# chenxy99/Scanpaths

Measured on AMD Instinct MI355X. Metric: images/sec/GPU (AiR train step, bs=32, 320x512) at 1/2/4/8 MI355X, higher is better.
Workload: dtype f32; 1 GPU; AiR supervised train step (fwd+loss+bwd+clip+Adam), resnet50, T=16, 320x512, per-GPU batch 32; global_batch=32, parallelism=dp1

## Files before the change

### scanpaths_amd/csrc/conv_f16x2.hip

```cpp
#include "common.h"
#include <algorithm>
#include <cstdlib>

typedef _Float16 f16x8 __attribute__((ext_vector_type(8)));

namespace {

#define SP_GLDS16(src, dst)                                                                                      \
    __builtin_amdgcn_global_load_lds((const __attribute__((address_space(1))) void*)(src),                       \
                                     (__attribute__((address_space(3))) void*)(dst), 16, 0, 0)

constexpr int HBM = 256, HBN = 128, HBK = 32;
constexpr int HA_BYTES = HBM * 128;
constexpr int HB_BYTES = HBN * 128;
constexpr int HSTAGE = HA_BYTES + HB_BYTES;
constexpr int HNSTAGE = 3;
constexpr int HCHUNK_KT = 8;
constexpr int HALO_W = 64, HALO_ROWSLOTS = HALO_W + 2, HALO_NSLOT = 6 * HALO_ROWSLOTS;
constexpr int HALO_PIECES = (HALO_NSLOT + 7) / 8;
constexpr int HALO_A_BYTES = HALO_PIECES * 1024;
constexpr int HALO_LDS = 2 * HALO_A_BYTES + 3 * HB_BYTES;

struct H2Args {
    const uint16_t* X;
    const uint16_t* W;
    const float* bias;
    float* C;
    const float* sx;
    const float* sw;
    int sw_rows;
    int64_t M;
    int Hi, Wi, Kc;
    int ldx;
    int Ho, Wo, Nout, ldc;
    int KH, KW, stride, pad, dil;
    int64_t ldwb;
    int64_t w_bstride;
    int rows_per_batch;
    int ncblk, nkt, tiles_n;
    float alpha;
    int beta, relu;
    uint32_t x_bytes, w_bytes;
    const float* l_xg;
    const float* l_cprev;
    const float* l_spcol;
    const float* l_wc;
    float* l_gates;
    float* l_c;
    float* l_h;
    unsigned* l_hamax;
    uint16_t* l_hplanes;
    float* l_hscale;
    float l_hbound;
    int lC, lP, lKP;
    int l_probe;
    double* st_partial;
    float* st_mm;
    const int* row_last;
    int row_step;
    int row_nimg;
};

__device__ __forceinline__ float h2_sigmoid(float x) { return sp_sigmoid(x); }
__device__ __forceinline__ int halo_swz(int slot) { return ((slot >> 1) & 3) << 1; }

template <int MODE, int NPROD, bool CBM, bool LSTM = false, bool HALO = false, int DBG = 0>
__global__ __launch_bounds__(512, 2) void h2_kernel(H2Args p) {
    static_assert(!LSTM || MODE == 0, "the LSTM epilogue belongs to the forward build");
    static_assert(!HALO || (CBM && NPROD == 3 && DBG == 0), "the halo build extends the channel-block-major schedule only");
    extern __shared__ __attribute__((aligned(16))) unsigned char smem[];
    constexpr bool LSTM_T = LSTM;
    const int t = threadIdx.x;
    const int lane = t & 63;
    const int wave = __builtin_amdgcn_readfirstlane(t >> 6);
    const int wm = wave >> 1, wn = wave & 1;

#ifdef SP_TIMING_VARIANTS
    const int probe = p.l_probe;
    if ((probe >> 8) && blockIdx.x < 256) {
        const int G = (probe >> 8) & 15, step_us = 2 * ((probe >> 12) & 31);
        const long long wait = (long long)((blockIdx.x >> 3) % G) * step_us * 100;
        const long long t0 = __builtin_amdgcn_s_memrealtime();
        while ((long long)__builtin_amdgcn_s_memrealtime() - t0 < wait) __builtin_amdgcn_s_sleep(32);
    }
#else
    constexpr int probe = 0;
#endif
    const float sx_dev = p.sx[0], sw_dev = p.sw_rows ? 1.f : p.sw[0];
    int tn, tmi;
    bool mapped = false;
    if constexpr (MODE == 1 && !LSTM) {
        if (p.row_nimg > 0) {
            const int mine = lane < p.row_nimg ? p.row_last[lane] : -1;
            const uint64_t lm = __ballot(lane < p.row_nimg && mine >= p.row_step);
            const uint64_t all = p.row_nimg == 64 ? ~0ull : ((1ull << p.row_nimg) - 1ull);
            const int tps = (p.Ho * p.Wo) / HBM;
            const int nlive = __popcll(lm);
            const int nl = nlive * tps * p.tiles_n;
            const int bid = blockIdx.x;
            uint64_t mask;
            int tml;
            if (bid < nl) {
                supertile_map(xcd_remap(bid, nl), nlive * tps, p.tiles_n, tml, tn, CBM);
                mask = lm;
            } else {
                tn = (bid - nl) % p.tiles_n;
                tml = (bid - nl) / p.tiles_n;
                mask = all & ~lm;
            }
            for (int k = tml / tps; k > 0; --k) mask &= mask - 1ull;
            tmi = (__ffsll((unsigned long long)mask) - 1) * tps + tml % tps;
            mapped = true;
        }
    }
    if (!mapped) supertile_map(xcd_remap(blockIdx.x, gridDim.x), gridDim.x / p.tiles_n, p.tiles_n, tmi, tn, CBM);
    const int64_t m0 = (int64_t)tmi * HBM;
    const int n0 = LSTM ? tn * 32 : tn * HBN;
    if constexpr (!LSTM) {
        if (p.row_last != nullptr) {
            const int howo = MODE == 1 ? p.Ho * p.Wo : p.rows_per_batch;
            const int img = (int)(m0 / howo);
            if (howo % HBM == 0 && m0 < p.M && p.row_last[img] < p.row_step) {
// ... 36 lines not shown
            a_px[j] = xo * p.stride - p.pad;
        } else {
            a_py[j] = yo + p.pad;
            a_px[j] = xo + p.pad;
        }
    }
    uint32_t b_voff[2];
    bool b_ok[2];
#pragma unroll
    for (int j = 0; j < 2; ++j) {
        const int idx = t + 512 * j;
        const int row = idx >> 3, pos = idx & 7;
        const int c8 = (pos ^ ((row >> 1) & 7)) * 16;
        if constexpr (LSTM) {
            const int ch = n0 + (row >> 6) * 16 + (row & 15);
            b_ok[j] = ch < p.lC;
            b_voff[j] = b_ok[j] ? (uint32_t)((int64_t)(((row >> 4) & 3) * p.lC + ch) * p.ldwb + c8) : 0u;
        } else {
            b_ok[j] = (n0 + row) < p.Nout;
            b_voff[j] = b_ok[j] ? (uint32_t)((int64_t)(n0 + row) * p.ldwb + c8) : 0u;
        }
    }
    const unsigned char* Wl = reinterpret_cast<const unsigned char*>(p.W);
    uint32_t w_left = p.w_bytes;
    if constexpr (!CBM) {
        if (p.w_bstride) {
            const int64_t off = (m0 / p.rows_per_batch) * p.w_bstride;
            Wl += off;
            w_left -= (uint32_t)off;
        }
    }
    int ld_ky = 0, ld_kx = 0, ld_cblk = 0, ld_kt = 0;
    uint32_t a_voff[4];
    bool a_ok[4];
    const int rowbytes = p.ldx * 4;
    uint32_t a_base0[4], a_mask[4];
    if constexpr (CBM && !HALO) {
#pragma unroll
        for (int j = 0; j < 4; ++j) {
            a_base0[j] = (uint32_t)(a_boff[j] + a_py[j] * p.Wi + a_px[j]) * (uint32_t)rowbytes + (uint32_t)a_c8[j];
            uint32_t msk = 0;
            for (int ky = 0; ky < p.KH; ++ky)
                for (int kx = 0; kx < p.KW; ++kx) {
                    const int iy = MODE == 0 ? a_py[j] + ky * p.dil : a_py[j] - ky * p.dil;
                    const int ix = MODE == 0 ? a_px[j] + kx * p.dil : a_px[j] - kx * p.dil;
                    if (a_rowok[j] && (unsigned)iy < (unsigned)p.Hi && (unsigned)ix < (unsigned)p.Wi) msk |= 1u << (ky * p.KW + kx);
                }
            a_mask[j] = msk;
        }
    }
    int ld_tap = 0;
    uint32_t h_off[7];
    uint32_t h_valid = 0;
    const int h_npieces = HALO ? (HALO_PIECES - wave + 7) / 8 : 0;
    if constexpr (HALO) {
        const int img = (int)((uint32_t)m0 / (uint32_t)HoWo);
        const int y0 = (int)(((uint32_t)m0 - (uint32_t)img * (uint32_t)HoWo) / (uint32_t)p.Wo);
#pragma unroll
        for (int j = 0; j < 7; ++j) {
            const int slot = (wave + 8 * j) * 8 + (lane >> 3), pos = lane & 7;
            const int br = slot / HALO_ROWSLOTS, sx = slot - br * HALO_ROWSLOTS;
            const int y = y0 - 1 + br, x = sx - 1;
            const bool ok = slot < HALO_NSLOT && (unsigned)y < (unsigned)p.Hi && (unsigned)x < (unsigned)p.Wi && m0 < p.M;
            h_off[j] = ok ? (uint32_t)((img * p.Hi + y) * p.Wi + x) * (uint32_t)rowbytes + (uint32_t)((pos ^ halo_swz(slot)) * 16) : 0u;
            h_valid |= ok ? (1u << j) : 0u;
        }
    }
    int h_cb = 0;
    auto issue_block = [&]() {
        if constexpr (HALO) {
            unsigned char* stA = smem + (h_cb & 1) * HALO_A_BYTES;
            const uint32_t koffA = (uint32_t)h_cb * 128u;
            const unsigned char* baseA = reinterpret_cast<const unsigned char*>(p.X) + koffA;
            const uint32_t zrelA = p.x_bytes - koffA;
#pragma unroll
            for (int j = 0; j < 7; ++j)
                if (j < h_npieces) SP_GLDS16(baseA + (((h_valid >> j) & 1u) ? h_off[j] : zrelA), stA + (wave + 8 * j) * 1024);
            ++h_cb;
        }
    };

    auto tap_update = [&]() {
#pragma unroll
        for (int j = 0; j < 4; ++j) {
            bool ok = a_rowok[j];
            int iy, ix;
            if (MODE == 0) {
                iy = a_py[j] + ld_ky * p.dil;
                ix = a_px[j] + ld_kx * p.dil;
                ok = ok && (unsigned)iy < (unsigned)p.Hi && (unsigned)ix < (unsigned)p.Wi;
            } else {
                const int ty = a_py[j] - ld_ky * p.dil, tx = a_px[j] - ld_kx * p.dil;
                ok = ok && ty >= 0 && tx >= 0;
                if (p.stride == 1) {
                    iy = ty;
                    ix = tx;
                } else {
                    iy = ty / p.stride;
                    ix = tx / p.stride;
                    ok = ok && (iy * p.stride == ty) && (ix * p.stride == tx);
                }
                ok = ok && iy < p.Hi && ix < p.Wi;
            }
            a_ok[j] = ok;
            a_voff[j] = ok ? (uint32_t)(a_boff[j] + iy * p.Wi + ix) * (uint32_t)rowbytes + (uint32_t)a_c8[j] : 0u;
        }
    };

    auto issue_tile = [&](int stage) {
        unsigned char* st = smem + stage * HSTAGE;
        if constexpr (HALO) {
            unsigned char* stB = smem + 2 * HALO_A_BYTES + stage * HB_BYTES;
            const uint32_t koffB = (uint32_t)(ld_tap * p.ncblk + ld_cblk) * 128u;
            const unsigned char* baseB = reinterpret_cast<const unsigned char*>(p.W) + koffB;
            const uint32_t zrelB = p.w_bytes - koffB;
#pragma unroll
            for (int j = 0; j < 2; ++j) SP_GLDS16(baseB + (b_ok[j] ? b_voff[j] : zrelB), stB + (wave + 8 * j) * 1024);
            if (++ld_tap == 9) {
                ld_tap = 0;
                ++ld_cblk;
            }
            return;
        }
        if constexpr (CBM) {
            const int step = (ld_ky * p.Wi + ld_kx) * p.dil;
            const uint32_t delta = (uint32_t)(MODE == 0 ? step : -step) * (uint32_t)rowbytes;
            const uint32_t koffA = (uint32_t)ld_cblk * 128u;
            const unsigned char* baseA = reinterpret_cast<const unsigned char*>(p.X) + koffA;
            const uint32_t zrelA = p.x_bytes - koffA;
#pragma unroll
            for (int j = 0; j < 4; ++j)
                SP_GLDS16(baseA + (((a_mask[j] >> ld_tap) & 1u) ? a_base0[j] + delta : zrelA), st + (wave + 8 * j) * 1024);
            const uint32_t koffB = (uint32_t)(ld_tap * p.ncblk + ld_cblk) * 128u;
            const unsigned char* baseB = reinterpret_cast<const unsigned char*>(p.W) + koffB;
            const uint32_t zrelB = p.w_bytes - koffB;
#pragma unroll
            for (int j = 0; j < 2; ++j) SP_GLDS16(baseB + (b_ok[j] ? b_voff[j] : zrelB), st + HA_BYTES + (wave + 8 * j) * 1024);
            ++ld_tap;
            if (++ld_kx == p.KW) {
                ld_kx = 0;
                if (++ld_ky == p.KH) {
                    ld_ky = 0;
                    ld_tap = 0;
                    ++ld_cblk;
                }
            }
            return;
        }
        if (ld_cblk == 0) tap_update();
        const uint32_t koffA = (uint32_t)ld_cblk * 128u;
        const unsigned char* baseA = reinterpret_cast<const unsigned char*>(p.X) + koffA;
        const uint32_t zrelA = p.x_bytes - koffA;
#pragma unroll
        for (int j = 0; j < 4; ++j) SP_GLDS16(baseA + (a_ok[j] ? a_voff[j] : zrelA), st + (wave + 8 * j) * 1024);
        const uint32_t koffB = (uint32_t)ld_kt * 128u;
        const unsigned char* baseB = Wl + koffB;
        const uint32_t zrelB = w_left - koffB;
#pragma unroll
        for (int j = 0; j < 2; ++j) SP_GLDS16(baseB + (b_ok[j] ? b_voff[j] : zrelB), st + HA_BYTES + (wave + 8 * j) * 1024);
        ++ld_kt;
        if (++ld_cblk == p.ncblk) {
            ld_cblk = 0;
            if (++ld_kx == p.KW) {
                ld_kx = 0;
                ++ld_ky;
            }
        }
    };

    const int l16 = lane & 15, g4 = lane >> 4;
    float pre_sw[4] = {1.f, 1.f, 1.f, 1.f};
    if constexpr (!LSTM && !HALO) {
        if (p.sw_rows) {
            int64_t r0 = 0;
            if constexpr (!CBM) {
                if (p.w_bstride) r0 = (m0 / p.rows_per_batch) * (int64_t)p.Nout;
            }
#pragma unroll
            for (int j = 0; j < 4; ++j) {
                const int n = n0 + wn * 64 + j * 16 + l16;
                if (n < p.Nout) pre_sw[j] = p.sw[r0 + n];
            }
        }
    }
    const int rot = (l16 >> 1) & 7;
    int offA[2], offB[2];
#pragma unroll
    for (int pl = 0; pl < 2; ++pl) {
        const int pos = ((g4 >> 1) * 4 + pl * 2 + (g4 & 1)) ^ rot;
        offA[pl] = (wm * 64 + l16) * 128 + pos * 16;
        offB[pl] = HA_BYTES + (wn * 64 + l16) * 128 + pos * 16;
    }

    const int h_slot0 = wm * HALO_ROWSLOTS + l16;
    const int h_chunk = (g4 >> 1) * 4 + (g4 & 1);
    int rd_tap = 0, rd_cb = 0;
    f32x4 tot4[4][4], acc4[4][4];
#pragma unroll
    for (int i = 0; i < 4; ++i)
#pragma unroll
        for (int j = 0; j < 4; ++j)
#pragma unroll
            for (int r = 0; r < 4; ++r) {
                tot4[i][j][r] = 0.f;
                acc4[i][j][r] = 0.f;
            }

    constexpr bool do_load = DBG != 1 && DBG != 3, do_mma = DBG != 2 && DBG != 9, do_lds = DBG != 3 && DBG != 9;
    constexpr bool do_bar = DBG != 3;
    int issued = 0;
    if constexpr (HALO) issue_block();
    if (do_load)
        for (; issued < HNSTAGE - 1 && issued < p.nkt; ++issued) issue_tile(issued);
    if (issued >= 2) {
        if constexpr (HALO) asm volatile("s_waitcnt vmcnt(2)" ::: "memory");
        else asm volatile("s_waitcnt vmcnt(6)" ::: "memory");
    } else {
        asm volatile("s_waitcnt vmcnt(0)" ::: "memory");
    }
    __builtin_amdgcn_s_barrier();

    f16x8 af[2][2][2], bf[2][2][2];
    auto read_frags = [&](int stage_, int kt_) {
        const unsigned char* st = smem + stage_ * HSTAGE;
        if constexpr (!do_lds) {
#pragma unroll
            for (int kk = 0; kk < 2; ++kk)
#pragma unroll
                for (int i = 0; i < 2; ++i)
#pragma unroll
                    for (int pl = 0; pl < 2; ++pl) {
                        f16x8 z;
#pragma unroll
                        for (int e = 0; e < 8; ++e) z[e] = (_Float16)(float)(kt_ + e + lane);
                        af[kk][i][pl] = z;
                        bf[kk][i][pl] = z;
                    }
        } else if constexpr (HALO) {
            const int ky = rd_tap / 3, kx = rd_tap - 3 * ky;
            const int slot = h_slot0 + (MODE == 0 ? ky * HALO_ROWSLOTS + kx : (2 - ky) * HALO_ROWSLOTS + 2 - kx);
            const int sw = halo_swz(slot);
            const unsigned char* stA = smem + (rd_cb & 1) * HALO_A_BYTES + slot * 128;
            const unsigned char* stB = smem + 2 * HALO_A_BYTES + stage_ * HB_BYTES - HA_BYTES;
            const int oa0 = ((h_chunk) ^ sw) * 16, oa1 = ((h_chunk + 2) ^ sw) * 16;
#pragma unroll
            for (int kk = 0; kk < 2; ++kk)
#pragma unroll
                for (int i = 0; i < 2; ++i) {
                    af[kk][i][0] = *reinterpret_cast<const f16x8*>(stA + oa0 + (2 * kk + i) * 16 * 128);
                    af[kk][i][1] = *reinterpret_cast<const f16x8*>(stA + oa1 + (2 * kk + i) * 16 * 128);
                    bf[kk][i][0] = *reinterpret_cast<const f16x8*>(stB + offB[0] + (2 * kk + i) * 16 * 128);
                    bf[kk][i][1] = *reinterpret_cast<const f16x8*>(stB + offB[1] + (2 * kk + i) * 16 * 128);
                }
            if (++rd_tap == 9) {
                rd_tap = 0;
                ++rd_cb;
            }
        } else {
#pragma unroll
            for (int kk = 0; kk < 2; ++kk)
#pragma unroll
                for (int i = 0; i < 2; ++i)
#pragma unroll
                    for (int pl = 0; pl < (NPROD == 3 ? 2 : 1); ++pl) {
                        af[kk][i][pl] = *reinterpret_cast<const f16x8*>(st + offA[pl] + (2 * kk + i) * 16 * 128);
                        bf[kk][i][pl] = *reinterpret_cast<const f16x8*>(st + offB[pl] + (2 * kk + i) * 16 * 128);
                    }
        }
    };
    auto mma_group = [&](int kk) {
        if constexpr (do_mma) {
#pragma unroll
            for (int i = 0; i < 2; ++i)
#pragma unroll
                for (int j = 0; j < 4; ++j) {
                    f32x4& a4 = acc4[2 * kk + i][j];
                    if constexpr (LSTM_T) {
                        if constexpr (NPROD == 3) {
                            a4 = __builtin_amdgcn_mfma_f32_16x16x32_f16(bf[j >> 1][j & 1][1], af[kk][i][0], a4, 0, 0, 0);
                            a4 = __builtin_amdgcn_mfma_f32_16x16x32_f16(bf[j >> 1][j & 1][0], af[kk][i][1], a4, 0, 0, 0);
                        }
                        a4 = __builtin_amdgcn_mfma_f32_16x16x32_f16(bf[j >> 1][j & 1][0], af[kk][i][0], a4, 0, 0, 0);
                        continue;
                    }
                    if constexpr (NPROD == 3) {
                        a4 = __builtin_amdgcn_mfma_f32_16x16x32_f16(af[kk][i][0], bf[j >> 1][j & 1][1], a4, 0, 0, 0);
                        a4 = __builtin_amdgcn_mfma_f32_16x16x32_f16(af[kk][i][1], bf[j >> 1][j & 1][0], a4, 0, 0, 0);
                    }
                    a4 = __builtin_amdgcn_mfma_f32_16x16x32_f16(af[kk][i][0], bf[j >> 1][j & 1][0], a4, 0, 0, 0);
                }
        } else {
#pragma unroll
            for (int i = 0; i < 2; ++i)
#pragma unroll
                for (int pl = 0; pl < 2; ++pl) {
                    const f16x8 x0 = af[kk][i][pl], x1 = bf[kk][i][pl];
                    asm volatile("" ::"v"(x0), "v"(x1));
                }
        }
    };
    auto fold = [&](int kt_) {
        if (((kt_ + 1) & (HCHUNK_KT - 1)) == 0) {
#pragma unroll
            for (int i = 0; i < 4; ++i)
#pragma unroll
                for (int j = 0; j < 4; ++j) {
                    tot4[i][j] += acc4[i][j];
#pragma unroll
                    for (int r = 0; r < 4; ++r) acc4[i][j][r] = 0.f;
                }
        }
    };
    auto wait_barrier = [&](int kt_) {
        if (kt_ + 2 < p.nkt) asm volatile("s_waitcnt vmcnt(6)" ::: "memory");
        else asm volatile("s_waitcnt vmcnt(0)" ::: "memory");
        asm volatile("s_waitcnt lgkmcnt(0)" ::: "memory");
        if constexpr (do_bar) __builtin_amdgcn_s_barrier();
    };
    auto prev_stage = [](int st_) { return st_ == 0 ? HNSTAGE - 1 : st_ - 1; };

    int stage = 0;
    const bool late = wave >= 4;
    if (late) __builtin_amdgcn_s_setprio(1);
    if constexpr (HALO) {
        int cur_tap = 0, cur_cb = 0;
        auto halo_issue = [&](int kt_) {
            if (kt_ + HNSTAGE - 1 < p.nkt) issue_tile(prev_stage(stage));
            if (cur_tap == 0 && cur_cb + 1 < p.ncblk) issue_block();
        };
        auto halo_wait = [&](int kt_) {
            if (kt_ + 2 < p.nkt) {
                if (cur_tap <= 1 && cur_cb + 1 < p.ncblk) {
                    if (h_npieces == 7) asm volatile("s_waitcnt vmcnt(9)" ::: "memory");
                    else asm volatile("s_waitcnt vmcnt(8)" ::: "memory");
                } else {
                    asm volatile("s_waitcnt vmcnt(2)" ::: "memory");
                }
            } else {
                asm volatile("s_waitcnt vmcnt(0)" ::: "memory");
            }
            asm volatile("s_waitcnt lgkmcnt(0)" ::: "memory");
            __builtin_amdgcn_s_barrier();
            if (++cur_tap == 9) {
                cur_tap = 0;
                ++cur_cb;
            }
        };
        if (!late) {
            for (int kt = 0; kt < p.nkt; ++kt) {
                read_frags(stage, kt);
                halo_issue(kt);
                mma_group(0);
                mma_group(1);
                fold(kt);
                halo_wait(kt);
                stage = (stage == HNSTAGE - 1) ? 0 : stage + 1;
            }
        } else {
            for (int kt = 0; kt < p.nkt; ++kt) {
                if (kt > 0) {
                    mma_group(0);
                    mma_group(1);
                    fold(kt - 1);
                }
                read_frags(stage, kt);
                halo_issue(kt);
                halo_wait(kt);
                stage = (stage == HNSTAGE - 1) ? 0 : stage + 1;
            }
            mma_group(0);
            mma_group(1);
            fold(p.nkt - 1);
        }
    } else if (!late) {
        for (int kt = 0; kt < p.nkt; ++kt) {
            const bool pre = do_load && kt + HNSTAGE - 1 < p.nkt;
            if (!CBM && pre) issue_tile(prev_stage(stage));
            read_frags(stage, kt);
            if (CBM && pre) issue_tile(prev_stage(stage));
            mma_group(0);
            mma_group(1);
            fold(kt);
            wait_barrier(kt);
            stage = (stage == HNSTAGE - 1) ? 0 : stage + 1;
        }
    } else {
        for (int kt = 0; kt < p.nkt; ++kt) {
            const bool pre = do_load && kt + HNSTAGE - 1 < p.nkt;
            if (kt > 0) {
                mma_group(0);
                mma_group(1);
                fold(kt - 1);
            }
            read_frags(stage, kt);
            if (pre) issue_tile(prev_stage(stage));
            wait_barrier(kt);
            stage = (stage == HNSTAGE - 1) ? 0 : stage + 1;
        }
        mma_group(0);
        mma_group(1);
        fold(p.nkt - 1);
    }
    if (late) __builtin_amdgcn_s_setprio(0);

    const float isx = 1.f / sx_dev, isw = 1.f / sw_dev;
    int64_t swrow0 = 0;
    if constexpr (!CBM) {
        if (p.w_bstride) swrow0 = (m0 / p.rows_per_batch) * (int64_t)p.Nout;
    }
    if constexpr (LSTM_T) {
        if (probe & 4) return;
        const bool nt_st = probe & 8, nt_ld = probe & 16;
        auto st4 = [&](float* dst, const float4& v) {
            const f32x4 x = {v.x, v.y, v.z, v.w};
            if (nt_st) __builtin_nontemporal_store(x, reinterpret_cast<f32x4*>(dst));
            else *reinterpret_cast<f32x4*>(dst) = x;
        };
        auto ld4 = [&](const float* src) {
            const f32x4 x = nt_ld ? __builtin_nontemporal_load(reinterpret_cast<const f32x4*>(src)) : *reinterpret_cast<const f32x4*>(src);
            return make_float4(x[0], x[1], x[2], x[3]);
        };
        const int KP = p.lKP, C = p.lC;
        const int b = (int)(m0 / p.lP);
        const int chb = n0 + wn * 16 + 4 * g4;
// ... 230 lines not shown
                    if (p.beta) {
                        const float4 o = *dst;
                        v.x += o.x; v.y += o.y; v.z += o.z; v.w += o.w;
                    }
                    if (p.relu) {
                        v.x = fmaxf(v.x, 0.f); v.y = fmaxf(v.y, 0.f); v.z = fmaxf(v.z, 0.f); v.w = fmaxf(v.w, 0.f);
                    }
                    *dst = v;
                }
            }
        }
        if (stats) {
            asm volatile("s_waitcnt lgkmcnt(0)" ::: "memory");
            __builtin_amdgcn_s_barrier();
            double* sh_s = reinterpret_cast<double*>(smem);
            float* sh_m = reinterpret_cast<float*>(smem + 4 * HBN * 2 * sizeof(double));
#pragma unroll
            for (int j = 0; j < 4; ++j) {
#pragma unroll
                for (int off = 16; off <= 32; off <<= 1) {
                    cs[j] += __shfl_xor(cs[j], off);
                    cq[j] += __shfl_xor(cq[j], off);
                    cmn[j] = fminf(cmn[j], __shfl_xor(cmn[j], off));
                    cmx[j] = fmaxf(cmx[j], __shfl_xor(cmx[j], off));
                }
                if (g4 == 0) {
                    const int col = wn * 64 + j * 16 + l16;
                    sh_s[(wm * HBN + col) * 2 + 0] = cs[j];
                    sh_s[(wm * HBN + col) * 2 + 1] = cq[j];
                    sh_m[(wm * HBN + col) * 2 + 0] = cmn[j];
                    sh_m[(wm * HBN + col) * 2 + 1] = cmx[j];
                }
            }
            asm volatile("s_waitcnt lgkmcnt(0)" ::: "memory");
            __builtin_amdgcn_s_barrier();
            if (t < HBN && n0 + t < p.Nout) {
                double a = 0.0, b = 0.0;
                float mn = INFINITY, mx = -INFINITY;
#pragma unroll
                for (int w = 0; w < 4; ++w) {
                    a += sh_s[(w * HBN + t) * 2 + 0];
                    b += sh_s[(w * HBN + t) * 2 + 1];
                    mn = fminf(mn, sh_m[(w * HBN + t) * 2 + 0]);
                    mx = fmaxf(mx, sh_m[(w * HBN + t) * 2 + 1]);
                }
                const int64_t g = m0 / HBM;
                p.st_partial[(g * 2 + 0) * p.Nout + n0 + t] = a;
                p.st_partial[(g * 2 + 1) * p.Nout + n0 + t] = b;
                p.st_mm[(g * 2 + 0) * p.Nout + n0 + t] = mn;
                p.st_mm[(g * 2 + 1) * p.Nout + n0 + t] = mx;
            }
        }
    }
}

struct HWArgs {
    const uint16_t* X;
    const uint16_t* dY;
    float* out;
    const float* sx;
    const float* sy;
    int sx_vec, sy_vec;
    int64_t M;
    int Hi, Wi, Ci, Ho, Wo, Co;
    int ldy;
    int Nvalid;
    int batched;
    int KH, KW, stride, pad, dil;
    int Ntot, ldo, tiles_n, splits;
    int64_t rows_per_split, slab_stride;
    float alpha;
    int beta;
    uint32_t x_bytes, y_bytes;
    const int* row_last;
    int row_step;
};

constexpr int HWA_ROW = 1024, HWB_ROW = 512;
constexpr int HWA_BYTES = 32 * HWA_ROW;
constexpr int HWB_BYTES = 32 * HWB_ROW;
constexpr int HWSTAGE = HWA_BYTES + HWB_BYTES;

typedef short short4v __attribute__((ext_vector_type(4)));

__device__ __forceinline__ f16x8 tr_pair_h(const unsigned char* base, int off0, int off1) {
    const short4v lo = __builtin_amdgcn_ds_read_tr16_b64_v4i16((__attribute__((address_space(3))) short4v*)(base + off0));
    const short4v hi = __builtin_amdgcn_ds_read_tr16_b64_v4i16((__attribute__((address_space(3))) short4v*)(base + off1));
    typedef short short8v __attribute__((ext_vector_type(8)));
    short8v v = __builtin_shufflevector(lo, hi, 0, 1, 2, 3, 4, 5, 6, 7);
    return __builtin_bit_cast(f16x8, v);
}

__device__ __forceinline__ int rot4(int q) { return 2 * (q & 1) + 8 * (q >> 1); }
__device__ __forceinline__ int swz16(int r) { return rot4(r & 3) + 4 * ((r >> 3) & 1); }
__device__ __forceinline__ int permA16(int j) { return ((j & 0x0c) << 2) | ((j & 0x30) >> 2) | (j & 3); }
__device__ __forceinline__ int permB16(int j) { return ((j & 0x0c) << 1) | ((j & 0x10) >> 2) | (j & 3); }
__device__ __forceinline__ int unpermB16(int x) { return ((x & 0x18) >> 1) | ((x & 0x04) << 2) | (x & 3); }

template <int NPROD, int DBG = 0>
__global__ __launch_bounds__(512, 2) void hw_kernel(HWArgs p) {
    constexpr bool do_load = DBG != 1 && DBG != 3 && DBG != 6, do_mma = DBG != 2 && DBG != 5 && DBG != 6, do_lds = DBG != 3 && DBG != 5 && DBG != 9;
    constexpr bool load_a = DBG != 8, load_b = DBG != 7;
    constexpr bool do_bar = DBG != 3;
    extern __shared__ __attribute__((aligned(16))) unsigned char smem[];
    const int t = threadIdx.x;
    const int lane = t & 63;
// ... 777 lines not shown
        const int c4 = c0 + cgi;
        float4 m = make_float4(0.f, 0.f, 0.f, 0.f);
        if (rr < rpb && c4 < C4)
            for (int64_t r = (int64_t)blockIdx.x * rpb + rr; r < rows; r += (int64_t)gridDim.x * rpb) {
                const float4 v = reinterpret_cast<const float4*>(x + r * C)[c4];
                m.x = fmaxf(m.x, fabsf(v.x)); m.y = fmaxf(m.y, fabsf(v.y)); m.z = fmaxf(m.z, fabsf(v.z)); m.w = fmaxf(m.w, fabsf(v.w));
            }
        __syncthreads();
        sh[threadIdx.x] = m;
        __syncthreads();
        if (rr == 0 && c4 < C4) {
            for (int k = 1; k < rpb; ++k) {
                const float4 o = sh[k * cg_per + cgi];
                m.x = fmaxf(m.x, o.x); m.y = fmaxf(m.y, o.y); m.z = fmaxf(m.z, o.z); m.w = fmaxf(m.w, o.w);
            }
            reinterpret_cast<float4*>(partial + (int64_t)blockIdx.x * C)[c4] = m;
        }
    }
}
__global__ __launch_bounds__(256) void colamax_final_kernel(const float* partial, int nblk, int C, float* col_scale) {
    __shared__ float sh[256];
    const int c = blockIdx.x * 32 + (threadIdx.x & 31), rg = threadIdx.x >> 5;
    float m = 0.f;
    if (c < C)
        for (int b = rg; b < nblk; b += 8) m = fmaxf(m, partial[(int64_t)b * C + c]);
    sh[threadIdx.x] = m;
    __syncthreads();
    if (rg == 0 && c < C) {
#pragma unroll
        for (int k = 1; k < 8; ++k) m = fmaxf(m, sh[k * 32 + (threadIdx.x & 31)]);
        col_scale[c] = m > 0.f ? scale_of(__float_as_uint(m)) : 0x1p100f;
    }
}

__global__ __launch_bounds__(256) void split2_cols_kernel(const float* x, int64_t n4, int C, const float* col_scale, uint16_t* out) {
    const int lane = threadIdx.x & 63;
    const int C4 = C / 4;
    const int64_t stride = (int64_t)gridDim.x * blockDim.x;
    for (int64_t base = (int64_t)blockIdx.x * blockDim.x + (threadIdx.x & ~63); base < n4; base += stride) {
        const int64_t i = base + lane;
        const bool live = i < n4;
        const float4 v = live ? reinterpret_cast<const float4*>(x)[i] : make_float4(0.f, 0.f, 0.f, 0.f);
        const float4 sc = live ? reinterpret_cast<const float4*>(col_scale)[i % C4] : make_float4(1.f, 1.f, 1.f, 1.f);
        ushort4 a, b;
        split2(v.x, sc.x, a.x, b.x);
        split2(v.y, sc.y, a.y, b.y);
        split2(v.z, sc.z, a.z, b.z);
        split2(v.w, sc.w, a.w, b.w);
        store_planes_quad(out, i, live, a, b);
    }
    if (blockIdx.x == 0 && threadIdx.x < 8) reinterpret_cast<uint2*>(out + 8 * n4)[threadIdx.x] = make_uint2(0u, 0u);
}

template <int MODE, int NPROD, bool CBM, bool LSTM = false, bool HALO = false, int DBG = 0>
int launch_h2(const H2Args& a, hipStream_t s) {
    auto kern = h2_kernel<MODE, NPROD, CBM, LSTM, HALO, DBG>;
    constexpr int lds = HALO ? HALO_LDS : HNSTAGE * HSTAGE;
    static bool attr_set = false;
    if (!attr_set) {
        (void)hipFuncSetAttribute(reinterpret_cast<const void*>(kern), hipFuncAttributeMaxDynamicSharedMemorySize, lds);
        attr_set = true;
    }
    const int64_t grid = sp_cdiv(a.M, HBM) * a.tiles_n;
    if (grid <= 0 || grid > 0x7fffffff) return SP_EINVAL;
    hipLaunchKernelGGL(kern, dim3((unsigned)grid), dim3(512), lds, s, a);
    SP_LAUNCH_CHECK();
    return SP_OK;
}

template <int NPROD, int DBG = 0>
int launch_hw(const HWArgs& a, int Co, hipStream_t s) {
    auto kern = hw_kernel<NPROD, DBG>;
    static bool attr_set = false;
    if (!attr_set) {
        (void)hipFuncSetAttribute(reinterpret_cast<const void*>(kern), hipFuncAttributeMaxDynamicSharedMemorySize, HNSTAGE * HWSTAGE);
        attr_set = true;
    }
    const int64_t grid = sp_cdiv(Co, 256) * a.tiles_n;
    hipLaunchKernelGGL(kern, dim3((unsigned)grid, (unsigned)a.splits), dim3(512), HNSTAGE * HWSTAGE, s, a);
    SP_LAUNCH_CHECK();
    return SP_OK;
}

int launch_amax(const float* x, int64_t n, unsigned* amax, hipStream_t s) {
    SP_RESET_AMAX(amax, s);
    const int64_t n4 = n / 4;
    const int blocks = (int)std::max<int64_t>(1, std::min<int64_t>(sp_cdiv(n4, 256 * 4), 1024));
    hipLaunchKernelGGL(amax_kernel, dim3(blocks), dim3(256), 0, s, x, n4, n, amax);
    SP_LAUNCH_CHECK();
    return SP_OK;
}

}

extern "C" int sp_split2_f16(const float* x, int64_t n, void* out, float* scale_amax, int have_amax, void* stream) {
    if (!x || !out || !scale_amax) return SP_ENULL;
    if (n % 16) return SP_EINVAL;
    hipStream_t s = (hipStream_t)stream;
    unsigned* amax = reinterpret_cast<unsigned*>(scale_amax + 1);
    if (!have_amax) {
        const int rc = launch_amax(x, n, amax, s);
        if (rc != SP_OK) return rc;
    }
    const int64_t n4 = n / 4;
    const int blocks = (int)std::max<int64_t>(1, std::min<int64_t>(sp_cdiv(n4, 256), 4096));
    hipLaunchKernelGGL(split2_kernel, dim3(blocks), dim3(256), 0, s, x, n4, amax, (uint16_t*)out, scale_amax);
    SP_LAUNCH_CHECK();
    return SP_OK;
}

extern "C" int sp_split2_f16_wT(const float* w, int Co, int taps, int Ci, void* out, float* scale_amax, void* stream) {
    if (!w || !out || !scale_amax) return SP_ENULL;
    if (((int64_t)taps * Co) % 16) return SP_EINVAL;
    hipStream_t s = (hipStream_t)stream;
    unsigned* amax = reinterpret_cast<unsigned*>(scale_amax + 1);
    const int64_t total = (int64_t)Co * taps * Ci;
    const int rc = launch_amax(w, total, amax, s);
    if (rc != SP_OK) return rc;
// ... 50 lines not shown
}

static bool halo_applies(const sp_conv_desc* d) {
    return d->KH == 3 && d->KW == 3 && d->stride == 1 && d->dil == 1 && d->pad == 1 && d->Wo == HALO_W && d->Wi == HALO_W &&
           d->Hi == d->Ho && (d->Ho * d->Wo) % HBM == 0 && d->Kc % 32 == 0;
}

static int conv_igemm_f16(const sp_conv_desc* d, const void* Xs, const float* x_scale, const void* Ws, const float* w_scale,
                          const float* bias, float* out, void* stream, int nprod, double* st_partial = nullptr,
                          float* st_mm = nullptr) {
    if (!d || !Xs || !Ws || !x_scale || !w_scale || !out) return SP_ENULL;
    if (d->mode != 0 && d->mode != 1) return SP_EINVAL;
    if (d->Kc % 32 || d->ldx < d->Kc || d->ldx % 16) return SP_EINVAL;
    if (((uintptr_t)Xs | (uintptr_t)Ws) & 15) return SP_EINVAL;
    if (d->nbatch < 1 || d->stride < 1 || d->dil < 1) return SP_EINVAL;
    const int64_t rows_b = (int64_t)d->N_img * d->Ho * d->Wo;
    if (d->nbatch > 1) {
        if (d->mode != 0 || d->KH * d->KW != 1 || d->stride != 1 || d->pad != 0 || rows_b % HBM || rows_b >= (1LL << 31)) return SP_EINVAL;
        if (d->strideX != rows_b * d->ldx || d->strideC != rows_b * d->ldc || d->strideW != (int64_t)d->Nout * d->Kc) return SP_EINVAL;
        if (st_partial || nprod != 3) return SP_EINVAL;
    }
    H2Args a{};
    a.X = (const uint16_t*)Xs; a.W = (const uint16_t*)Ws; a.bias = bias; a.C = out;
    a.sx = x_scale; a.sw = w_scale; a.sw_rows = d->w_scale_rows ? 1 : 0;
    a.row_last = ((d->mode == 1 && d->nbatch == 1) || (d->mode == 0 && d->nbatch > 1)) ? d->row_last : nullptr; a.row_step = d->row_step;
    a.row_nimg = (a.row_last && d->mode == 1 && d->nbatch == 1 && d->N_img <= 64 && ((int64_t)d->Ho * d->Wo) % HBM == 0 &&
                  sp_tuning_get(SP_TUNE_ROW_ORDER, 1) == 1) ? d->N_img : 0;
    a.M = rows_b * d->nbatch;
    a.Hi = d->Hi; a.Wi = d->Wi; a.Kc = d->Kc; a.ldx = d->ldx;
    a.Ho = d->Ho; a.Wo = d->Wo; a.Nout = d->Nout; a.ldc = d->ldc;
    a.KH = d->KH; a.KW = d->KW; a.stride = d->stride; a.pad = d->pad; a.dil = d->dil;
    a.w_bstride = d->nbatch > 1 ? 4 * d->strideW : 0;
    a.rows_per_batch = (int)rows_b;
    a.ldwb = 4 * (int64_t)d->KH * d->KW * d->Kc;
    a.ncblk = d->Kc / 32;
    a.nkt = d->KH * d->KW * a.ncblk;
    a.tiles_n = (int)sp_cdiv(d->Nout, HBN);
    a.alpha = d->alpha; a.beta = d->beta; a.relu = d->relu;
    const int64_t xb = 4LL * d->nbatch * d->N_img * d->Hi * d->Wi * d->ldx, wb = 4LL * d->nbatch * d->Nout * d->KH * d->KW * d->Kc;
    if (xb + 64 >= (1LL << 32) || wb + 64 >= (1LL << 32)) return SP_EINVAL;
    a.x_bytes = (uint32_t)xb; a.w_bytes = (uint32_t)wb;
    if (a.M <= 0 || a.M >= (1LL << 31) || a.Nout <= 0) return SP_EINVAL;
    hipStream_t st = (hipStream_t)stream;
    const bool f = d->mode == 0;
    const bool cbm_ok = d->KH * d->KW > 1 && d->KH * d->KW <= 32 && (f || d->stride == 1);
    if (st_partial) {
        if (!f || !st_mm || nprod != 3 || d->beta || d->relu || bias) return SP_EINVAL;
        a.st_partial = st_partial; a.st_mm = st_mm;
        return cbm_ok ? launch_h2<0, 3, true>(a, st) : launch_h2<0, 3, false>(a, st);
    }
#ifdef SP_TIMING_VARIANTS
    if (sp_tuning_get(SP_TUNE_H2_DBG, 0) >= 256) a.l_probe = sp_tuning_get(SP_TUNE_H2_DBG, 0) & ~255;
    switch (sp_tuning_get(SP_TUNE_H2_DBG, 0)) {
        case 6: return f ? launch_h2<0, 3, false, false, false, 1>(a, st) : launch_h2<1, 3, false, false, false, 1>(a, st);
        case 7: return f ? launch_h2<0, 3, false, false, false, 2>(a, st) : launch_h2<1, 3, false, false, false, 2>(a, st);
        case 8: return f ? launch_h2<0, 3, false, false, false, 3>(a, st) : launch_h2<1, 3, false, false, false, 3>(a, st);
        case 9: return f ? launch_h2<0, 3, false, false, false, 9>(a, st) : launch_h2<1, 3, false, false, false, 9>(a, st);
        default: break;
    }
#endif
    if (nprod == 1)
        return f ? launch_h2<0, 1, false>(a, st) : launch_h2<1, 1, false>(a, st);
    if (cbm_ok && halo_applies(d) && sp_tuning_get(SP_TUNE_H2_HALO, 1) == 1)
        return f ? launch_h2<0, 3, true, false, true>(a, st) : launch_h2<1, 3, true, false, true>(a, st);
    if (cbm_ok) return f ? launch_h2<0, 3, true>(a, st) : launch_h2<1, 3, true>(a, st);
    return f ? launch_h2<0, 3, false>(a, st) : launch_h2<1, 3, false>(a, st);
}

extern "C" int sp_conv_igemm_f16x2(const sp_conv_desc* d, const void* Xs, const float* x_scale, const void* Ws,
                                   const float* w_scale, const float* bias, float* out, void* stream) {
    return conv_igemm_f16(d, Xs, x_scale, Ws, w_scale, bias, out, stream, 3);
}

extern "C" int64_t sp_conv_stats_tiles(const sp_conv_desc* d) {
    if (!d) return 0;
    return sp_cdiv((int64_t)d->N_img * d->Ho * d->Wo, HBM);
}
extern "C" int sp_conv_igemm_f16x2_stats(const sp_conv_desc* d, const void* Xs, const float* x_scale, const void* Ws,
                                         const float* w_scale, float* out, double* st_partial, float* st_mm, void* stream) {
    if (!st_partial || !st_mm) return SP_ENULL;
    return conv_igemm_f16(d, Xs, x_scale, Ws, w_scale, nullptr, out, stream, 3, st_partial, st_mm);
}

extern "C" int sp_conv_igemm_f16x1(const sp_conv_desc* d, const void* Xs, const float* x_scale, const void* Ws,
                                   const float* w_scale, const float* bias, float* out, void* stream) {
    return conv_igemm_f16(d, Xs, x_scale, Ws, w_scale, bias, out, stream, 1);
}

extern "C" int sp_gateconv_lstm_f16x2(const sp_conv_desc* d, const void* Hs, const float* h_scale, const void* Ws,
                                      const float* w_scale, const float* xg, const float* c_prev, const float* spcol,
                                      const float* wc, int P, int KP, float* gates, float* c_out, float* h_out, unsigned* h_amax,
                                      void* hout_planes, float* hout_scale, float hout_bound, void* stream) {
    if (!d || !Hs || !Ws || !h_scale || !w_scale || !xg || !spcol || !wc || !gates || !c_out || !h_out) return SP_ENULL;
    if (d->mode != 0 || d->Kc % 32 || d->ldx != d->Kc || d->nbatch != 1 || d->stride != 1 || d->dil < 1) return SP_EINVAL;
    if (d->Nout != 4 * d->Kc || d->Ho != d->Hi || d->Wo != d->Wi || d->KH * d->KW < 2 || d->KH * d->KW > 32) return SP_EINVAL;
    if (P != d->Ho * d->Wo || P % HBM || KP < 1 || KP > 32) return SP_EINVAL;
    if (((uintptr_t)Hs | (uintptr_t)Ws) & 15) return SP_EINVAL;
    if (((uintptr_t)xg | (uintptr_t)c_prev | (uintptr_t)gates | (uintptr_t)c_out | (uintptr_t)h_out) & 15) return SP_EINVAL;
    if (d->w_scale_rows && ((uintptr_t)w_scale & 15)) return SP_EINVAL;
    H2Args a{};
    a.X = (const uint16_t*)Hs; a.W = (const uint16_t*)Ws; a.bias = nullptr; a.C = nullptr;
    a.sx = h_scale; a.sw = w_scale; a.sw_rows = d->w_scale_rows ? 1 : 0;
    a.M = (int64_t)d->N_img * P;
    a.Hi = d->Hi; a.Wi = d->Wi; a.Kc = d->Kc; a.ldx = d->Kc;
    a.Ho = d->Ho; a.Wo = d->Wo; a.Nout = d->Nout; a.ldc = d->Nout;
    a.KH = d->KH; a.KW = d->KW; a.stride = 1; a.pad = d->pad; a.dil = d->dil;
    a.ldwb = 4 * (int64_t)d->KH * d->KW * d->Kc;
    a.ncblk = d->Kc / 32;
    a.nkt = d->KH * d->KW * a.ncblk;
    a.tiles_n = d->Kc / 32;
    a.alpha = 1.f; a.beta = 0; a.relu = 0;
    const int64_t xb = 4LL * a.M * d->Kc, wb = 4LL * d->Nout * d->KH * d->KW * d->Kc;
    if (xb + 64 >= (1LL << 32) || wb + 64 >= (1LL << 32) || a.M <= 0) return SP_EINVAL;
    a.x_bytes = (uint32_t)xb; a.w_bytes = (uint32_t)wb;
    a.l_xg = xg; a.l_cprev = c_prev; a.l_spcol = spcol; a.l_wc = wc;
    if (hout_planes && (!hout_scale || !(hout_bound > 0.f) || ((uintptr_t)hout_planes & 15))) return SP_EINVAL;
    a.l_gates = gates; a.l_c = c_out; a.l_h = h_out; a.l_hamax = h_amax;
    a.l_hplanes = (uint16_t*)hout_planes; a.l_hscale = hout_scale; a.l_hbound = hout_bound;
    a.lC = d->Kc; a.lP = P; a.lKP = KP;
    a.l_probe = sp_tuning_get(SP_TUNE_H2_DBG, 0);
    hipStream_t st = (hipStream_t)stream;
    SP_RESET_AMAX(h_amax, st);
    if (halo_applies(d) && sp_tuning_get(SP_TUNE_H2_HALO, 1) == 1) return launch_h2<0, 3, true, true, true>(a, st);
    return launch_h2<0, 3, true, true, false>(a, st);
}

extern "C" int64_t sp_conv_wgrad_f16x2_workspace(const sp_wgrad_desc* d) {
    if (!d) return 0;
    if (d->nbatch > 1) return 0;
    const int sp = hw_splits(d);
    return sp <= 1 ? 0 : (int64_t)sp * d->Co * d->ldo * (int64_t)sizeof(float);
}

static int launch_hw_reduce(const HWScales& sc, const float* slab, float* dW, int Co, int Ntot, int ldo, int splits, int64_t slab_stride,
                            float alpha, int beta, hipStream_t s) {
    const int64_t total = (int64_t)Co * Ntot;
    if (Ntot % 4 == 0 && ldo % 4 == 0 && slab_stride % 4 == 0 && sc.Ci % 4 == 0 && (((uintptr_t)slab | (uintptr_t)dW) & 15) == 0) {
        const int blocks = (int)std::min<int64_t>(sp_cdiv(total / 4, 256), 4096);
        hipLaunchKernelGGL(hw_reduce4_kernel, dim3(blocks), dim3(256), 0, s, slab, dW, Co, Ntot / 4, ldo / 4, splits, slab_stride / 4, alpha, sc, beta);
    } else {
        const int blocks = (int)std::min<int64_t>(sp_cdiv(total, 256), 4096);
        hipLaunchKernelGGL(hw_reduce_kernel, dim3(blocks), dim3(256), 0, s, slab, dW, Co, Ntot, ldo, splits, slab_stride, alpha, sc, beta);
    }
    SP_LAUNCH_CHECK();
    return SP_OK;
}

static int conv_wgrad_f16(const sp_wgrad_desc* d, const void* Xsplit, const float* x_scale, const void* dYsplit,
                          const float* y_scale, float* dW, void* workspace, void* stream, int nprod) {
    if (!d || !Xsplit || !dYsplit || !x_scale || !y_scale || !dW) return SP_ENULL;
    if (d->Ci % 16 || d->Co % 16 || d->ldx != d->Ci || d->ldy < d->Co || d->ldy % 16 || d->nbatch < 1) return SP_EINVAL;
    if (((uintptr_t)Xsplit | (uintptr_t)dYsplit) & 15) return SP_EINVAL;
    const int64_t rows_b = (int64_t)d->N_img * d->Ho * d->Wo;
    const bool batched = d->nbatch > 1;
    if (batched) {
        if (d->KH * d->KW != 1 || d->stride != 1 || d->pad != 0 || rows_b % 32 || nprod != 3) return SP_EINVAL;
        if (d->strideX != rows_b * d->Ci || d->strideY != rows_b * d->ldy || d->strideO != (int64_t)d->Co * d->ldo) return SP_EINVAL;
    } else if (d->ldo < d->KH * d->KW * d->Ci) {
        return SP_EINVAL;
    }
    HWArgs a;
    a.X = (const uint16_t*)Xsplit; a.dY = (const uint16_t*)dYsplit;
    a.sx = x_scale; a.sy = y_scale;
    a.sx_vec = d->x_scale_vec ? 1 : 0; a.sy_vec = d->y_scale_vec ? 1 : 0;
    if (batched && (a.sx_vec || a.sy_vec)) return SP_EINVAL;
    a.row_last = batched ? d->row_last : nullptr; a.row_step = d->row_step;
    a.M = rows_b * d->nbatch;
    a.Hi = d->Hi; a.Wi = d->Wi; a.Ci = d->Ci; a.Ho = d->Ho; a.Wo = d->Wo; a.Co = d->Co; a.ldy = d->ldy;
    a.KH = d->KH; a.KW = d->KW; a.stride = d->stride; a.pad = d->pad; a.dil = d->dil;
    a.Ntot = d->KH * d->KW * d->Ci;
    a.ldo = d->ldo;
    a.tiles_n = (int)sp_cdiv(a.Ntot, 128);
    a.Nvalid = std::min(a.Ntot, d->ldo);
    a.batched = batched ? 1 : 0;
    a.splits = batched ? d->nbatch : hw_splits(d);
    if (!batched && a.splits > 1 && !workspace) return SP_ENULL;
    a.rows_per_split = batched ? rows_b : sp_cdiv(sp_cdiv(a.M, a.splits), 32) * 32;
// ... 115 lines not shown
```

Baseline: 144.2 images/s.

## Add 4-stage weight ring halo conv kernel by dropping halo edge slots

Adds a RING4 variant of the halo implicit-GEMM conv kernel. It shrinks the activation halo tile from 66 to 64 slots per row, masking the edge columns with zeroed fragments in registers. The saved LDS pays for a fourth weight pipeline stage with retuned vmcnt waits. It is launched by default for the forward mode when the device LDS limit allows, otherwise the 3-stage kernel runs as fallback. The risks are higher LDS use per block, which may limit occupancy, and correctness at the tile edges now resting on the register masking.

```diff
diff --git a/scanpaths_amd/csrc/conv_f16x2.hip b/scanpaths_amd/csrc/conv_f16x2.hip
--- a/scanpaths_amd/csrc/conv_f16x2.hip
+++ b/scanpaths_amd/csrc/conv_f16x2.hip
@@ -20,6 +20,11 @@
 constexpr int HALO_PIECES = (HALO_NSLOT + 7) / 8;
 constexpr int HALO_A_BYTES = HALO_PIECES * 1024;
 constexpr int HALO_LDS = 2 * HALO_A_BYTES + 3 * HB_BYTES;
+constexpr int HALO4_NSLOT = 6 * HALO_W;
+constexpr int HALO4_PIECES = HALO4_NSLOT / 8;
+constexpr int HALO4_A_BYTES = HALO4_PIECES * 1024;
+constexpr int HALO4_NSTAGE = 4;
+constexpr int HALO4_LDS = 2 * HALO4_A_BYTES + HALO4_NSTAGE * HB_BYTES;
 
 struct H2Args {
     const uint16_t* X;
@@ -64,10 +69,14 @@
 __device__ __forceinline__ float h2_sigmoid(float x) { return sp_sigmoid(x); }
 __device__ __forceinline__ int halo_swz(int slot) { return ((slot >> 1) & 3) << 1; }
 
-template <int MODE, int NPROD, bool CBM, bool LSTM = false, bool HALO = false, int DBG = 0>
-__global__ __launch_bounds__(512, 2) void h2_kernel(H2Args p) {
+template <int MODE, int NPROD, bool CBM, bool LSTM, bool HALO, int DBG, bool RING4>
+__device__ __forceinline__ void h2_body(const H2Args& p) {
     static_assert(!LSTM || MODE == 0, "the LSTM epilogue belongs to the forward build");
     static_assert(!HALO || (CBM && NPROD == 3 && DBG == 0), "the halo build extends the channel-block-major schedule only");
+    static_assert(!RING4 || HALO, "the 4-stage weight ring belongs to the halo build");
+    constexpr int H_ROWSLOTS = RING4 ? HALO_W : HALO_ROWSLOTS, H_NSLOT = 6 * H_ROWSLOTS, H_XOFF = RING4 ? 0 : 1;
+    constexpr int H_MAXP = RING4 ? 6 : 7, H_A_BYTES = RING4 ? HALO4_A_BYTES : HALO_A_BYTES;
+    constexpr int NSTG = RING4 ? HALO4_NSTAGE : HNSTAGE;
     extern __shared__ __attribute__((aligned(16))) unsigned char smem[];
     constexpr bool LSTM_T = LSTM;
     const int t = threadIdx.x;
@@ -210,16 +219,16 @@
     int ld_tap = 0;
     uint32_t h_off[7];
     uint32_t h_valid = 0;
-    const int h_npieces = HALO ? (HALO_PIECES - wave + 7) / 8 : 0;
+    const int h_npieces = !HALO ? 0 : RING4 ? 6 : (HALO_PIECES - wave + 7) / 8;
     if constexpr (HALO) {
         const int img = (int)((uint32_t)m0 / (uint32_t)HoWo);
         const int y0 = (int)(((uint32_t)m0 - (uint32_t)img * (uint32_t)HoWo) / (uint32_t)p.Wo);
 #pragma unroll
         for (int j = 0; j < 7; ++j) {
             const int slot = (wave + 8 * j) * 8 + (lane >> 3), pos = lane & 7;
-            const int br = slot / HALO_ROWSLOTS, sx = slot - br * HALO_ROWSLOTS;
-            const int y = y0 - 1 + br, x = sx - 1;
-            const bool ok = slot < HALO_NSLOT && (unsigned)y < (unsigned)p.Hi && (unsigned)x < (unsigned)p.Wi && m0 < p.M;
+            const int br = slot / H_ROWSLOTS, sx = slot - br * H_ROWSLOTS;
+            const int y = y0 - 1 + br, x = sx - H_XOFF;
+            const bool ok = j < H_MAXP && slot < H_NSLOT && (unsigned)y < (unsigned)p.Hi && (unsigned)x < (unsigned)p.Wi && m0 < p.M;
             h_off[j] = ok ? (uint32_t)((img * p.Hi + y) * p.Wi + x) * (uint32_t)rowbytes + (uint32_t)((pos ^ halo_swz(slot)) * 16) : 0u;
             h_valid |= ok ? (1u << j) : 0u;
         }
@@ -227,12 +236,12 @@
     int h_cb = 0;
     auto issue_block = [&]() {
         if constexpr (HALO) {
-            unsigned char* stA = smem + (h_cb & 1) * HALO_A_BYTES;
+            unsigned char* stA = smem + (h_cb & 1) * H_A_BYTES;
             const uint32_t koffA = (uint32_t)h_cb * 128u;
             const unsigned char* baseA = reinterpret_cast<const unsigned char*>(p.X) + koffA;
             const uint32_t zrelA = p.x_bytes - koffA;
 #pragma unroll
-            for (int j = 0; j < 7; ++j)
+            for (int j = 0; j < H_MAXP; ++j)
                 if (j < h_npieces) SP_GLDS16(baseA + (((h_valid >> j) & 1u) ? h_off[j] : zrelA), stA + (wave + 8 * j) * 1024);
             ++h_cb;
         }
@@ -268,7 +277,7 @@
     auto issue_tile = [&](int stage) {
         unsigned char* st = smem + stage * HSTAGE;
         if constexpr (HALO) {
-            unsigned char* stB = smem + 2 * HALO_A_BYTES + stage * HB_BYTES;
+            unsigned char* stB = smem + 2 * H_A_BYTES + stage * HB_BYTES;
             const uint32_t koffB = (uint32_t)(ld_tap * p.ncblk + ld_cblk) * 128u;
             const unsigned char* baseB = reinterpret_cast<const unsigned char*>(p.W) + koffB;
             const uint32_t zrelB = p.w_bytes - koffB;
@@ -350,7 +359,7 @@
         offB[pl] = HA_BYTES + (wn * 64 + l16) * 128 + pos * 16;
     }
 
-    const int h_slot0 = wm * HALO_ROWSLOTS + l16;
+    const int h_slot0 = wm * H_ROWSLOTS + l16;
     const int h_chunk = (g4 >> 1) * 4 + (g4 & 1);
     int rd_tap = 0, rd_cb = 0;
     f32x4 tot4[4][4], acc4[4][4];
@@ -369,8 +378,10 @@
     int issued = 0;
     if constexpr (HALO) issue_block();
     if (do_load)
-        for (; issued < HNSTAGE - 1 && issued < p.nkt; ++issued) issue_tile(issued);
-    if (issued >= 2) {
+        for (; issued < NSTG - 1 && issued < p.nkt; ++issued) issue_tile(issued);
+    if (RING4 && issued >= 3) {
+        asm volatile("s_waitcnt vmcnt(4)" ::: "memory");
+    } else if (issued >= 2) {
         if constexpr (HALO) asm volatile("s_waitcnt vmcnt(2)" ::: "memory");
         else asm volatile("s_waitcnt vmcnt(6)" ::: "memory");
     } else {
@@ -379,6 +390,7 @@
     __builtin_amdgcn_s_barrier();
 
     f16x8 af[2][2][2], bf[2][2][2];
+    bool m_lo = false, m_hi = false;
     auto read_frags = [&](int stage_, int kt_) {
         const unsigned char* st = smem + stage_ * HSTAGE;
         if constexpr (!do_lds) {
@@ -394,6 +406,31 @@
                         af[kk][i][pl] = z;
                         bf[kk][i][pl] = z;
                     }
+        } else if constexpr (RING4) {
+            const int ky = rd_tap / 3, kx = rd_tap - 3 * ky;
+            const int dy = MODE == 0 ? ky : 2 - ky, dx = MODE == 0 ? kx : 2 - kx;
+            const int s1 = h_slot0 + dy * H_ROWSLOTS + dx + 15;
+            const bool zlo = dx == 0 && l16 == 0, zhi = dx == 2 && l16 == 15;
+            const int sw = halo_swz(s1);
+            const int sl[4] = {zlo ? s1 : s1 - 16, s1, s1 + 16, zhi ? s1 + 16 : s1 + 32};
+            const unsigned char* stA = smem + (rd_cb & 1) * H_A_BYTES;
+            const unsigned char* stB = smem + 2 * H_A_BYTES + stage_ * HB_BYTES - HA_BYTES;
+            const int oa0 = ((h_chunk) ^ sw) * 16, oa1 = ((h_chunk + 2) ^ sw) * 16;
+#pragma unroll
+            for (int kk = 0; kk < 2; ++kk)
+#pragma unroll
+                for (int i = 0; i < 2; ++i) {
+                    af[kk][i][0] = *reinterpret_cast<const f16x8*>(stA + sl[2 * kk + i] * 128 + oa0);
+                    af[kk][i][1] = *reinterpret_cast<const f16x8*>(stA + sl[2 * kk + i] * 128 + oa1);
+                    bf[kk][i][0] = *reinterpret_cast<const f16x8*>(stB + offB[0] + (2 * kk + i) * 16 * 128);
+                    bf[kk][i][1] = *reinterpret_cast<const f16x8*>(stB + offB[1] + (2 * kk + i) * 16 * 128);
+                }
+            m_lo = zlo;
+            m_hi = zhi;
+            if (++rd_tap == 9) {
+                rd_tap = 0;
+                ++rd_cb;
+            }
         } else if constexpr (HALO) {
             const int ky = rd_tap / 3, kx = rd_tap - 3 * ky;
             const int slot = h_slot0 + (MODE == 0 ? ky * HALO_ROWSLOTS + kx : (2 - ky) * HALO_ROWSLOTS + 2 - kx);
@@ -457,6 +494,20 @@
                 }
         }
     };
+    auto halo_mma = [&]() {
+        const f16x8 zero = {0, 0, 0, 0, 0, 0, 0, 0};
+        if constexpr (RING4) {
+#pragma unroll
+            for (int pl = 0; pl < 2; ++pl) af[0][0][pl] = m_lo ? zero : af[0][0][pl];
+        }
+        mma_group(0);
+        if constexpr (RING4) {
+            __builtin_amdgcn_sched_barrier(0);
+#pragma unroll
+            for (int pl = 0; pl < 2; ++pl) af[1][1][pl] = m_hi ? zero : af[1][1][pl];
+        }
+        mma_group(1);
+    };
     auto fold = [&](int kt_) {
         if (((kt_ + 1) & (HCHUNK_KT - 1)) == 0) {
 #pragma unroll
@@ -475,7 +526,7 @@
         asm volatile("s_waitcnt lgkmcnt(0)" ::: "memory");
         if constexpr (do_bar) __builtin_amdgcn_s_barrier();
     };
-    auto prev_stage = [](int st_) { return st_ == 0 ? HNSTAGE - 1 : st_ - 1; };
+    auto prev_stage = [](int st_) { return st_ == 0 ? NSTG - 1 : st_ - 1; };
 
     int stage = 0;
     const bool late = wave >= 4;
@@ -483,11 +534,20 @@
     if constexpr (HALO) {
         int cur_tap = 0, cur_cb = 0;
         auto halo_issue = [&](int kt_) {
-            if (kt_ + HNSTAGE - 1 < p.nkt) issue_tile(prev_stage(stage));
+            if (kt_ + NSTG - 1 < p.nkt) issue_tile(prev_stage(stage));
             if (cur_tap == 0 && cur_cb + 1 < p.ncblk) issue_block();
         };
         auto halo_wait = [&](int kt_) {
-            if (kt_ + 2 < p.nkt) {
+            if constexpr (RING4) {
+                if (kt_ + 3 < p.nkt) {
+                    if (cur_tap <= 2 && cur_cb + 1 < p.ncblk) asm volatile("s_waitcnt vmcnt(10)" ::: "memory");
+                    else asm volatile("s_waitcnt vmcnt(4)" ::: "memory");
+                } else if (kt_ + 2 < p.nkt) {
+                    asm volatile("s_waitcnt vmcnt(2)" ::: "memory");
+                } else {
+                    asm volatile("s_waitcnt vmcnt(0)" ::: "memory");
+                }
+            } else if (kt_ + 2 < p.nkt) {
                 if (cur_tap <= 1 && cur_cb + 1 < p.ncblk) {
                     if (h_npieces == 7) asm volatile("s_waitcnt vmcnt(9)" ::: "memory");
                     else asm volatile("s_waitcnt vmcnt(8)" ::: "memory");
@@ -508,26 +568,23 @@
             for (int kt = 0; kt < p.nkt; ++kt) {
                 read_frags(stage, kt);
                 halo_issue(kt);
-                mma_group(0);
-                mma_group(1);
+                halo_mma();
                 fold(kt);
                 halo_wait(kt);
-                stage = (stage == HNSTAGE - 1) ? 0 : stage + 1;
+                stage = (stage == NSTG - 1) ? 0 : stage + 1;
             }
         } else {
             for (int kt = 0; kt < p.nkt; ++kt) {
                 if (kt > 0) {
-                    mma_group(0);
-                    mma_group(1);
+                    halo_mma();
                     fold(kt - 1);
                 }
                 read_frags(stage, kt);
                 halo_issue(kt);
                 halo_wait(kt);
-                stage = (stage == HNSTAGE - 1) ? 0 : stage + 1;
-            }
-            mma_group(0);
-            mma_group(1);
+                stage = (stage == NSTG - 1) ? 0 : stage + 1;
+            }
+            halo_mma();
             fold(p.nkt - 1);
         }
     } else if (!late) {
@@ -864,6 +921,15 @@
             }
         }
     }
+}
+
+template <int MODE, int NPROD, bool CBM, bool LSTM = false, bool HALO = false, int DBG = 0>
+__global__ __launch_bounds__(512, 2) void h2_kernel(H2Args p) {
+    h2_body<MODE, NPROD, CBM, LSTM, HALO, DBG, false>(p);
+}
+template <int MODE, bool LSTM>
+__global__ __launch_bounds__(512, 2) void h2_halo4_kernel(H2Args p) {
+    h2_body<MODE, 3, true, LSTM, true, 0, true>(p);
 }
 
 struct HWArgs {
@@ -1747,10 +1813,10 @@
     if (blockIdx.x == 0 && threadIdx.x < 8) reinterpret_cast<uint2*>(out + 8 * n4)[threadIdx.x] = make_uint2(0u, 0u);
 }
 
-template <int MODE, int NPROD, bool CBM, bool LSTM = false, bool HALO = false, int DBG = 0>
+template <int MODE, int NPROD, bool CBM, bool LSTM = false, int DBG = 0>
 int launch_h2(const H2Args& a, hipStream_t s) {
-    auto kern = h2_kernel<MODE, NPROD, CBM, LSTM, HALO, DBG>;
-    constexpr int lds = HALO ? HALO_LDS : HNSTAGE * HSTAGE;
+    auto kern = h2_kernel<MODE, NPROD, CBM, LSTM, false, DBG>;
+    constexpr int lds = HNSTAGE * HSTAGE;
     static bool attr_set = false;
     if (!attr_set) {
         (void)hipFuncSetAttribute(reinterpret_cast<const void*>(kern), hipFuncAttributeMaxDynamicSharedMemorySize, lds);
@@ -1759,6 +1825,37 @@
     const int64_t grid = sp_cdiv(a.M, HBM) * a.tiles_n;
     if (grid <= 0 || grid > 0x7fffffff) return SP_EINVAL;
     hipLaunchKernelGGL(kern, dim3((unsigned)grid), dim3(512), lds, s, a);
+    SP_LAUNCH_CHECK();
+    return SP_OK;
+}
+
+template <int MODE, bool LSTM>
+int launch_h2_halo(const H2Args& a, hipStream_t s) {
+#ifdef SP_TIMING_VARIANTS
+    constexpr bool built4 = true;
+#else
+    constexpr bool built4 = MODE == 0;
+#endif
+    auto kern4 = h2_halo4_kernel<built4 ? MODE : 0, LSTM>;
+    auto kern3 = h2_kernel<MODE, 3, true, LSTM, true, 0>;
+    static int ring4 = -1;
+    if (ring4 < 0) {
+        int dev = 0, max_lds = 0;
+        ring4 = hipGetDevice(&dev) == hipSuccess &&
+                hipDeviceGetAttribute(&max_lds, hipDeviceAttributeMaxSharedMemoryPerBlock, dev) == hipSuccess && max_lds >= HALO4_LDS &&
+                hipFuncSetAttribute(reinterpret_cast<const void*>(kern4), hipFuncAttributeMaxDynamicSharedMemorySize, HALO4_LDS) == hipSuccess;
+        (void)hipGetLastError();
+        (void)hipFuncSetAttribute(reinterpret_cast<const void*>(kern3), hipFuncAttributeMaxDynamicSharedMemorySize, HALO_LDS);
+    }
+    const int64_t grid = sp_cdiv(a.M, HBM) * a.tiles_n;
+    if (grid <= 0 || grid > 0x7fffffff) return SP_EINVAL;
+    const int knob = sp_tuning_get(SP_TUNE_H2_HALO, 1);
+    if (built4 && ring4 == 1 && knob != 3 && (MODE == 0 || knob == 4)) {
+        hipLaunchKernelGGL(kern4, dim3((unsigned)grid), dim3(512), HALO4_LDS, s, a);
+        if (hipGetLastError() == hipSuccess) return SP_OK;
+        ring4 = 0;
+    }
+    hipLaunchKernelGGL(kern3, dim3((unsigned)grid), dim3(512), HALO_LDS, s, a);
     SP_LAUNCH_CHECK();
     return SP_OK;
 }
@@ -1915,17 +2012,17 @@
 #ifdef SP_TIMING_VARIANTS
     if (sp_tuning_get(SP_TUNE_H2_DBG, 0) >= 256) a.l_probe = sp_tuning_get(SP_TUNE_H2_DBG, 0) & ~255;
     switch (sp_tuning_get(SP_TUNE_H2_DBG, 0)) {
-        case 6: return f ? launch_h2<0, 3, false, false, false, 1>(a, st) : launch_h2<1, 3, false, false, false, 1>(a, st);
-        case 7: return f ? launch_h2<0, 3, false, false, false, 2>(a, st) : launch_h2<1, 3, false, false, false, 2>(a, st);
-        case 8: return f ? launch_h2<0, 3, false, false, false, 3>(a, st) : launch_h2<1, 3, false, false, false, 3>(a, st);
-        case 9: return f ? launch_h2<0, 3, false, false, false, 9>(a, st) : launch_h2<1, 3, false, false, false, 9>(a, st);
+        case 6: return f ? launch_h2<0, 3, false, false, 1>(a, st) : launch_h2<1, 3, false, false, 1>(a, st);
+        case 7: return f ? launch_h2<0, 3, false, false, 2>(a, st) : launch_h2<1, 3, false, false, 2>(a, st);
+        case 8: return f ? launch_h2<0, 3, false, false, 3>(a, st) : launch_h2<1, 3, false, false, 3>(a, st);
+        case 9: return f ? launch_h2<0, 3, false, false, 9>(a, st) : launch_h2<1, 3, false, false, 9>(a, st);
         default: break;
     }
 #endif
     if (nprod == 1)
         return f ? launch_h2<0, 1, false>(a, st) : launch_h2<1, 1, false>(a, st);
-    if (cbm_ok && halo_applies(d) && sp_tuning_get(SP_TUNE_H2_HALO, 1) == 1)
-        return f ? launch_h2<0, 3, true, false, true>(a, st) : launch_h2<1, 3, true, false, true>(a, st);
+    if (cbm_ok && halo_applies(d) && sp_tuning_get(SP_TUNE_H2_HALO, 1) != 0)
+        return f ? launch_h2_halo<0, false>(a, st) : launch_h2_halo<1, false>(a, st);
     if (cbm_ok) return f ? launch_h2<0, 3, true>(a, st) : launch_h2<1, 3, true>(a, st);
     return f ? launch_h2<0, 3, false>(a, st) : launch_h2<1, 3, false>(a, st);
 }
@@ -1984,8 +2081,8 @@
     a.l_probe = sp_tuning_get(SP_TUNE_H2_DBG, 0);
     hipStream_t st = (hipStream_t)stream;
     SP_RESET_AMAX(h_amax, st);
-    if (halo_applies(d) && sp_tuning_get(SP_TUNE_H2_HALO, 1) == 1) return launch_h2<0, 3, true, true, true>(a, st);
-    return launch_h2<0, 3, true, true, false>(a, st);
+    if (halo_applies(d) && sp_tuning_get(SP_TUNE_H2_HALO, 1) != 0) return launch_h2_halo<0, true>(a, st);
+    return launch_h2<0, 3, true, true>(a, st);
 }
 
 extern "C" int64_t sp_conv_wgrad_f16x2_workspace(const sp_wgrad_desc* d) {
```

After: 141.5 images/s. -1.9%, worse.
